# TravisWheelerLab/BATH

Measured on NVIDIA B200. Metric: frameshift Forward GCUPS, higher is better.
Workload: dtype f32

## Files before the change

### bath_b200/csrc/bathgpu.cu

```cuda
#include <cuda_runtime.h>
#include <stdint.h>
#include <stdio.h>
#include <stdarg.h>
#include <string.h>
#include <stdlib.h>
#include <math.h>
#include <thread>
#include <vector>
#include <string>
#include <algorithm>
#include <mutex>
#include <memory>

#include "../../include/bathgpu.h"
#include "fs_parser.cuh"
#include "fs_parser_v3.cuh"
#include "fs_backward.cuh"
#include "fs_domain.cuh"
#include "orf_domain.cuh"
#include "orf_filters.cuh"
#include "orf_finder.cuh"
#include "bias_filter.cuh"
#include "microbench.cuh"
#include "launch.h"
// ... 29 lines not shown
      if (ms >= 1.0) fprintf(stderr, "[bathgpu] device buffer %zu -> %zu bytes: %.2f ms\n", old, want, ms);
    }
    return BATHGPU_OK;
  }
  void release() { if (p) cudaFree(p); p = nullptr; cap = 0; }
  template <class T> T *as() const { return reinterpret_cast<T *>(p); }
};

struct FsProfileImage {
  int   which = 0, M = 0, nrows = 0, J = 0, mpad = 0, scan_steps = 5;
  DevBuf emis;
  DevBuf emis_bck, cellb3;
  DevBuf cellbmw;
  DevBuf emis_fwd;
  DevBuf cellc;
  DevBuf cellmw;
  int    mw_scan_steps = 5;
  DevBuf cellb;
  DevBuf cellf5;
  DevBuf amino;
  DevBuf oaflags;
  DevBuf oapass;
  DevBuf tfvraw;
  DevBuf zinv;
  bool  loaded = false;
};

struct FsProfileSet {
  int n = 0;
  std::vector<int> J, scan_steps, mw_scan_steps;
// ... 412 lines not shown
          for (int lane = 0; lane < 32; ++lane) {
            mw[(size_t)(5 * JW + s2) * VL + 32 * w + lane] = (lane >= d) ? (float)bsw[lane] : 0.0f;
            if (lane >= d) { biggest = std::max(biggest, bw[lane]); nbs[lane] = bsw[lane] * bsw[lane - d]; nb[lane] = bw[lane] * bw[lane - d]; }
          }
          bsw.swap(nbs); bw.swap(nb);
          if (biggest < 1.0e-9 && need == 5) need = std::max(s2, 3);
        }
        mw_scan_steps = std::max(mw_scan_steps, need);
      }
      if (getenv("BATHGPU_FULL_SCAN")) mw_scan_steps = 5;
    } else mw.clear();
    if (getenv("BATHGPU_FULL_SCAN")) scan_steps = 5;
  }
}

static void fs5_forward_consts(const Fold &f, std::vector<float> &cc)
{
  const int M = f.M, J = f.J;
  const std::vector<double> &sK = f.sK, &zK = f.zK;
  auto T = [&](int t, int k) -> double { return f.T(t, k); };
  cc.assign((size_t)(F5_COUNT * J + 5) * 32, 0.0f);
  auto C = [&](int which_c, int j, int lane) -> float & { return cc[(size_t)(which_c * J + j) * 32 + lane]; };
  std::vector<double> bfull(32, 1.0);
  for (int lane = 0; lane < 32; ++lane) {
    double pp = 1.0;
    for (int j = 0; j < J; ++j) {
      int k = lane * J + j + 1;
      if (k <= M) {
        double sn = sK[k + 1];
        C(F5_MM, j, lane) = (float)(T(tMM, k) / (zK[k] * sn));
// ... 42 lines not shown

  {
    std::vector<float> ef, cc, mw;
    forward3_tables(f, which, nrows, rfv, ef, cc, mw, im.scan_steps, im.mw_scan_steps);
    if (im.emis_fwd.reserve(ef.size() * sizeof(float)) != BATHGPU_OK) return fail(ctx, BATHGPU_EMEM, "device allocation failed");
    CUDA_TRY(ctx, cudaMemcpyAsync(im.emis_fwd.p, ef.data(), ef.size() * sizeof(float), cudaMemcpyHostToDevice, ctx->stream));
    CUDA_TRY(ctx, wait_stream(ctx));
    if (!mw.empty()) {
      if (im.cellmw.reserve(mw.size() * sizeof(float)) != BATHGPU_OK) return fail(ctx, BATHGPU_EMEM, "device allocation failed");
      CUDA_TRY(ctx, cudaMemcpyAsync(im.cellmw.p, mw.data(), mw.size() * sizeof(float), cudaMemcpyHostToDevice, ctx->stream));
      CUDA_TRY(ctx, wait_stream(ctx));
    } else im.cellmw.release();
    if (im.cellc.reserve(cc.size() * sizeof(float)) != BATHGPU_OK) return fail(ctx, BATHGPU_EMEM, "device allocation failed");
    CUDA_TRY(ctx, cudaMemcpyAsync(im.cellc.p, cc.data(), cc.size() * sizeof(float), cudaMemcpyHostToDevice, ctx->stream));
    CUDA_TRY(ctx, wait_stream(ctx));
  }

  {
    std::vector<float> cc((size_t)(BC_COUNT * J + BL_COUNT) * 32, 0.0f);
    auto C = [&](int which_c, int j, int lane) -> float & { return cc[(size_t)(which_c * J + j) * 32 + lane]; };
    std::vector<double> bfull(32, 1.0);
    for (int lane = 0; lane < 32; ++lane) {
      double pp = 1.0;
      for (int j = 0; j < J; ++j) {
        int k = lane * J + j + 1;
        if (k <= M) {
          double sn = sK[k + 1];
          C(BC_VMM, j, lane) = (float)(T(tMM, k) / (sn * zK[k]));
          C(BC_VIM, j, lane) = (float)(T(tIM, k) / sn);
          C(BC_VDM, j, lane) = (float)(T(tDM, k) / sn);
// ... 333 lines not shown
    return fail(ctx, BATHGPU_EMEM, "device allocation failed for a %lld-nt block", n);
  if (!A.bytes_valid) {
    unpack_dna4_kernel<<<(unsigned)(((n + 7) / 8 + 255) / 256), 256, 0, ctx->stream>>>(A.dna4.as<uint32_t>(), n, A.dna_bytes.as<uint8_t>());
    A.bytes_valid = true;
  }
  revcomp_kernel<<<(unsigned)((n + 255) / 256), 256, 0, ctx->stream>>>(A.dna_bytes.as<uint8_t>(), n, B.dna_bytes.as<uint8_t>());
  pack_dna4_kernel<<<(unsigned)((nwords + 255) / 256), 256, 0, ctx->stream>>>(B.dna_bytes.as<uint8_t>(), n, B.dna4.as<uint32_t>(), nwords);
  CUDA_TRY(ctx, cudaGetLastError());
  CUDA_TRY(ctx, wait_stream(ctx));
  B.block_n = n; B.nres = 0; B.bytes_valid = true;
  return BATHGPU_OK;
}


static cudaError_t dispatch_fwd(bool xmx, int J, const FsParserArgs &a, int sms, cudaStream_t s);

static int fs_fwd_block_impl(bathgpu_ctx *ctx, const uint8_t *dsq, const uint8_t *packed, int64_t n, const bathgpu_window *wins, int nwin,
                             const float xfE[2], float *fwdsc, int32_t *status)
{
  if (!ctx || (!dsq && !packed) || n < 1 || !wins || nwin < 1 || !xfE || !fwdsc || !status) return fail(ctx, BATHGPU_EINVAL, "bad arguments to bathgpu_fs_fwd_block");
  if (!ctx->fs3.loaded) return fail(ctx, BATHGPU_EINVAL, "3-codon profile not loaded");
  for (int w = 0; w < nwin; ++w)
    if (wins[w].L < 3 || wins[w].start < 1 || wins[w].start + wins[w].L - 1 > n)
      return fail(ctx, BATHGPU_EINVAL, "window %d (start %lld, L %d) is outside the block (n=%lld) or shorter than 3", w, (long long)wins[w].start, wins[w].L, (long long)n);
  CUDA_TRY(ctx, enter(ctx));
  if (!ctx->copy_stream) {
    CUDA_TRY(ctx, cudaStreamCreateWithFlags(&ctx->copy_stream, cudaStreamNonBlocking));
    CUDA_TRY(ctx, cudaStreamCreateWithFlags(&ctx->stream2, cudaStreamNonBlocking));
    for (auto &e : ctx->chunk_ev) CUDA_TRY(ctx, cudaEventCreateWithFlags(&e, cudaEventDisableTiming));
  }
// ... 54 lines not shown
  int w0 = 0, launches = 0;
  for (int c = 0; c < K; ++c) {
    const long long ready_nt = (c == K - 1) ? n : 8 * (cuts[c] / 8);
    int w1 = w0;
    while (w1 < nwin && hw[w1].start + hw[w1].L - 1 <= ready_nt) ++w1;
    if (c == K - 1) w1 = nwin;
    if (w1 == w0) continue;
    cudaStream_t s = (launches & 1) ? ctx->stream2 : ctx->stream;
    if (launches == 1) CUDA_TRY(ctx, cudaStreamWaitEvent(ctx->stream2, ctx->ev0, 0));
    CUDA_TRY(ctx, cudaStreamWaitEvent(s, pack_ev[c], 0));
    FsParserArgs a{};
    a.emis = im.emis_fwd.as<float>(); a.cellc = im.cellc.as<float>(); a.dna4 = S.dna4.as<uint32_t>();
    a.wins = ctx->wins.as<WindowDesc>() + w0; a.nwin = w1 - w0; a.mpad = im.mpad; a.tEM = xfE[0]; a.tEL = xfE[1];
    a.fwdsc = ctx->fwdsc.as<float>() + w0; a.status = ctx->status.as<int>() + w0; a.xmx = nullptr; a.xoff = nullptr;
    a.counter = ctx->counter.as<int>() + launches; a.scan_steps = im.scan_steps; a.cellmw = im.cellmw.as<float>(); a.mw_scan_steps = im.mw_scan_steps;
    CUDA_TRY(ctx, dispatch_fwd(false, im.J, a, ctx->prop.multiProcessorCount, s));
    ++launches;
    w0 = w1;
  }
  if (launches > 1) {
    CUDA_TRY(ctx, cudaEventRecord(join_ev[0], ctx->stream2));
    CUDA_TRY(ctx, cudaStreamWaitEvent(ctx->stream, join_ev[0], 0));
  }
  CUDA_TRY(ctx, cudaEventRecord(ctx->ev1, ctx->stream));
  CUDA_TRY(ctx, cudaMemcpyAsync(in_order ? fwdsc : sc.data(), ctx->fwdsc.p, (size_t)nwin * 4, cudaMemcpyDeviceToHost, ctx->stream));
  CUDA_TRY(ctx, cudaMemcpyAsync(in_order ? status : st.data(), ctx->status.p, (size_t)nwin * 4, cudaMemcpyDeviceToHost, ctx->stream));
  CUDA_TRY(ctx, wait_stream(ctx));
  CUDA_TRY(ctx, cudaStreamSynchronize(ctx->copy_stream));
  if (!in_order) for (int w = 0; w < nwin; ++w) { fwdsc[order[w]] = sc[w]; status[order[w]] = st[w]; }
  CUDA_TRY(ctx, cudaEventElapsedTime(&ctx->last_ms, ctx->ev0, ctx->ev1));
// ... 8 lines not shown
  if (!dsq) return fail(ctx, BATHGPU_EINVAL, "bad arguments to bathgpu_fs_fwd_block");
  return fs_fwd_block_impl(ctx, dsq, nullptr, n, wins, nwin, xfE, fwdsc, status);
}

extern "C" int bathgpu_fs_fwd_block_packed4(bathgpu_ctx *ctx, const uint8_t *packed, int64_t n, const bathgpu_window *wins, int nwin,
                                            const float xfE[2], float *fwdsc, int32_t *status)
{
  if (!packed) return fail(ctx, BATHGPU_EINVAL, "bad arguments to bathgpu_fs_fwd_block_packed4");
  return fs_fwd_block_impl(ctx, nullptr, packed, n, wins, nwin, xfE, fwdsc, status);
}

static int fwd_version(int J)
{
  static const int forced = [] { const char *e = getenv("BATHGPU_FWD"); int x = e ? atoi(e) : 0; return (x == 3 || x == 4) ? x : 0; }();
  if (forced) return forced;
  return (J == 10) ? 4 : 3;
}

static cudaError_t dispatch_fwd(bool xmx, int J, const FsParserArgs &a, int sms, cudaStream_t s)
{
  cudaError_t e = cudaErrorInvalidValue;
  const int v = fwd_version(J);
#define X(S) if (launch_fs3_forward_##S(J, xmx, v, a, sms, s, &e)) return e;
  BATHGPU_FOR_EACH_SET(X)
#undef X
  return cudaErrorInvalidValue;
}

static int check_windows(bathgpu_ctx *ctx, const bathgpu_window *wins, int n)
{
  for (int w = 0; w < n; ++w) {
// ... 22 lines not shown
}

extern "C" int bathgpu_fs_fwd_staged(bathgpu_ctx *ctx, const float xfE[2])
{
  if (!ctx || !xfE)          return fail(ctx, BATHGPU_EINVAL, "bad arguments to bathgpu_fs_fwd_staged");
  if (!ctx->fs3.loaded)      return fail(ctx, BATHGPU_EINVAL, "3-codon profile not loaded");
  if (ctx->nstaged < 1)      return fail(ctx, BATHGPU_EINVAL, "no windows staged");
  CUDA_TRY(ctx, enter(ctx));
  const FsProfileImage &im = ctx->fs3;
  FsParserArgs a{};
  a.emis = im.emis_fwd.as<float>(); a.cellc = im.cellc.as<float>(); a.dna4 = ctx->S().dna4.as<uint32_t>();
  a.wins = ctx->wins.as<WindowDesc>(); a.nwin = ctx->nstaged; a.mpad = im.mpad;
  a.tEM = xfE[0]; a.tEL = xfE[1];
  a.fwdsc = ctx->fwdsc.as<float>(); a.status = ctx->status.as<int>();
  a.xmx = nullptr; a.xoff = nullptr; a.counter = ctx->counter.as<int>(); a.scan_steps = im.scan_steps; a.cellmw = im.cellmw.as<float>(); a.mw_scan_steps = im.mw_scan_steps;

  CUDA_TRY(ctx, cudaMemsetAsync(ctx->counter.p, 0, 4, ctx->stream));
  CUDA_TRY(ctx, cudaEventRecord(ctx->ev0, ctx->stream));
  CUDA_TRY(ctx, dispatch_fwd(false, im.J, a, ctx->prop.multiProcessorCount, ctx->stream));
  CUDA_TRY(ctx, cudaEventRecord(ctx->ev1, ctx->stream));
  CUDA_TRY(ctx, wait_stream(ctx));
  CUDA_TRY(ctx, cudaEventElapsedTime(&ctx->last_ms, ctx->ev0, ctx->ev1));
  ctx->last_launches = 1;
  return BATHGPU_OK;
}

extern "C" int bathgpu_fetch_scores(bathgpu_ctx *ctx, float *fwdsc, int32_t *status, int n)
{
  if (!ctx || n < 1 || n > ctx->nstaged) return fail(ctx, BATHGPU_EINVAL, "bad arguments to bathgpu_fetch_scores");
  CUDA_TRY(ctx, enter(ctx));
// ... 41 lines not shown
      ctx->dmocc.reserve(rows * 4) != BATHGPU_OK || ctx->dbtot.reserve(rows * 4) != BATHGPU_OK || ctx->detot.reserve(rows * 4) != BATHGPU_OK)
    return fail(ctx, BATHGPU_EMEM, "device allocation failed for %d windows (%zu rows)", n, rows);
  CUDA_TRY(ctx, cudaMemcpyAsync(ctx->wins.p, wins, (size_t)n * sizeof(WindowDesc), cudaMemcpyHostToDevice, ctx->stream));
  CUDA_TRY(ctx, cudaMemcpyAsync(ctx->xoff.p, xoff.data(), (size_t)(n + 1) * 8, cudaMemcpyHostToDevice, ctx->stream));
  ctx->nstaged = n;
  ctx->xrows = (int64_t)rows;

  const int sms = ctx->prop.multiProcessorCount;
  CUDA_TRY(ctx, cudaEventRecord(ctx->ev0, ctx->stream));

  FsParserArgs fa{};
  fa.emis = im.emis_fwd.as<float>(); fa.cellc = im.cellc.as<float>(); fa.dna4 = ctx->S().dna4.as<uint32_t>();
  fa.wins = ctx->wins.as<WindowDesc>(); fa.nwin = n; fa.mpad = im.mpad; fa.tEM = xfE[0]; fa.tEL = xfE[1];
  fa.fwdsc = ctx->fwdsc.as<float>(); fa.status = ctx->status.as<int>();
  fa.xmx = ctx->fxmx.as<float>(); fa.xoff = ctx->xoff.as<long long>(); fa.counter = ctx->counter.as<int>(); fa.scan_steps = im.scan_steps; fa.cellmw = im.cellmw.as<float>(); fa.mw_scan_steps = im.mw_scan_steps;
  CUDA_TRY(ctx, cudaMemsetAsync(ctx->counter.p, 0, 4, ctx->stream));
  CUDA_TRY(ctx, dispatch_fwd(true, im.J, fa, sms, ctx->stream));

  FsBackwardArgs ba{};
  ba.emis = im.emis_bck.as<float>(); ba.cellb = im.cellb3.as<float>(); ba.cellbmw = im.cellbmw.as<float>(); ba.dna4 = fa.dna4; ba.wins = fa.wins; ba.nwin = n; ba.mpad = im.mpad;
  ba.tEM = xfE[0]; ba.tEL = xfE[1]; ba.fxmx = ctx->fxmx.as<float>(); ba.bxmx = ctx->bxmx.as<float>(); ba.xoff = fa.xoff;
  ba.bcksc = ctx->bcksc.as<float>(); ba.status = fa.status; ba.counter = fa.counter;
  CUDA_TRY(ctx, cudaMemsetAsync(ctx->counter.p, 0, 4, ctx->stream));
  CUDA_TRY(ctx, dispatch_bck(im.J, ba, sms, ctx->stream));

  std::vector<float> hm, hb, he;
  if (decode) {
    DomainDecodeArgs da{};
    da.fxmx = ba.fxmx; da.bxmx = ba.bxmx; da.xoff = fa.xoff; da.wins = fa.wins; da.nwin = n;
    da.tNL = xf5_loop[0]; da.tJL = xf5_loop[1]; da.tCL = xf5_loop[2];
// ... 1208 lines not shown
```

### bath_b200/csrc/fs_parser.cuh

```cuda
#pragma once
#include <cuda_runtime.h>
#include <stdint.h>

namespace bathgpu {

constexpr int kWarp = 32;

enum FwdCellConst { FC_MM = 0, FC_DM, FC_MD, FC_DD, FC_MI, FC_II, FC_COUNT };
enum FwdLaneConst { FL_B0 = 0, FL_B1, FL_B2, FL_B3, FL_B4, FL_COUNT };

struct WindowDesc {
  long long start;
  int       L;
  float     pmove;
  float     ploop;
};

struct FsSetProfile {
  const float *emis;
  const float *cellc;
  const float *cellmw;
  float        tEM, tEL;
};

// ... 3 lines not shown
  const uint32_t *dna4;
  const WindowDesc *wins;
  int             nwin;
  int             mpad;
  float           tEM, tEL;
  float          *fwdsc;
  int            *status;
  float          *xmx;
  const long long *xoff;
  int            *counter;
  int             scan_steps;
  const float    *cellmw;
  int             mw_scan_steps;
  const FsSetProfile *set;
  const int      *wprof;
};

template <int J> struct VecOf { static constexpr int V = (J % 4 == 0) ? 4 : ((J % 2 == 0) ? 2 : 1); };

__device__ __forceinline__ int codon2_fs3(int w, int x)               { int c = x * 84 + w * 21;                 return min(c, 337); }
__device__ __forceinline__ int codon3_fs3(int v, int w, int x)        { int c = x * 84 + w * 21 + v * 5 + 1;     return min(c, 336); }
__device__ __forceinline__ int codon4_fs3(int u, int v, int w, int x) { int c = x * 84 + w * 21 + v * 5 + u + 2; return min(c, 337); }

template <int J, int VEC>
__device__ __forceinline__ void load_emission_row(const float *__restrict__ row, float (&e)[J])
{
#pragma unroll
  for (int g = 0; g < J / VEC; ++g) {
    if constexpr (VEC == 4) {
      float4 t = __ldg(reinterpret_cast<const float4 *>(row) + g * kWarp);
// ... 185 lines not shown
```

### bath_b200/csrc/fs_parser_v3.cuh

```cuda
#pragma once
#include "fs_parser.cuh"

#ifndef BATHGPU_V3_JOINT_E
#define BATHGPU_V3_JOINT_E(J) (((J) >= 2 && (J) <= 5) || (J) == 8)
#endif

namespace bathgpu {

struct RowOut { float xE, xN, xJ, xC, xB, scale; };

template <int J, int VEC, int PH, int NS, bool HEAD>
__device__ __forceinline__ void fwd_row_compute(int i, int lane, FwdState<J> &S, const FwdConsts<J> &K,
                                                const char *__restrict__ emis_lane, unsigned rowbytes, uint32_t cw,
                                                float ploop, float pmove, float tEL, float tEM, RowOut &R)
{
  constexpr int P0 = PH, P1 = (PH + 3) & 3, P2 = (PH + 2) & 3, P3 = (PH + 1) & 3;
  float e2[J], e3[J], e4[J], m[J];
  load_emission_row<J, VEC>(reinterpret_cast<const float *>(emis_lane + (size_t)(cw & 511u) * rowbytes), e2);
  load_emission_row<J, VEC>(reinterpret_cast<const float *>(emis_lane + (size_t)((cw >> 9) & 511u) * rowbytes), e3);
  load_emission_row<J, VEC>(reinterpret_cast<const float *>(emis_lane + (size_t)(cw >> 18) * rowbytes), e4);

  float es0 = 0.f, es1 = 0.f;
#pragma unroll
  for (int j = 0; j < J; ++j) {
    float t = S.W[P2][j] * e4[j];
    t = fmaf(S.W[P1][j], e3[j], t);
    t = fmaf(S.W[P0][j], e2[j], t);
    m[j] = t;
    if (j == 0) es0 = t * K.qm[0]; else if (j == 1) es1 = t * K.qm[1]; else if (j & 1) es1 = fmaf(t, K.qm[j], es1); else es0 = fmaf(t, K.qm[j], es0);
  }
  float xE = warp_allsum(J > 1 ? es0 + es1 : es0);

  float A = 0.f;
#pragma unroll
  for (int j = 0; j < J; ++j) A = (j == 0) ? m[0] : fmaf(A, K.dd[j], m[j]);
// ... 17 lines not shown
    o[j] = fmaf(d, K.dm[j], t);
    if (j + 1 < J) d = fmaf(d, K.dd[j], m[j]);
    S.I[P1][j] = fmaf(S.I[P0][j], K.ii[j], m[j]);
  }
  float oprev = __shfl_up_sync(0xffffffffu, o[J - 1], 1);
  if (lane == 0) oprev = 0.f;
  S.W[P2][0] = xB + oprev;
#pragma unroll
  for (int j = 1; j < J; ++j) S.W[P2][j] = xB + o[j - 1];
  S.xN[P0] = xN; S.xJ[P0] = xJ; S.xC[P0] = xC;
  R.xE = xE; R.xN = xN; R.xJ = xJ; R.xC = xC; R.xB = xB; R.scale = 1.0f;
}

template <int J> struct RowMid { float m[J]; float es, d; };

template <int J, int VEC, int PH, int NS>
__device__ __forceinline__ void fwd_row_front(const FwdState<J> &S, const FwdConsts<J> &K, const char *__restrict__ emis_lane, unsigned rowbytes,
                                              uint32_t cw, RowMid<J> &X)
{
  constexpr int P0 = PH, P1 = (PH + 3) & 3, P2 = (PH + 2) & 3;
  float e2[J], e3[J], e4[J];
  load_emission_row<J, VEC>(reinterpret_cast<const float *>(emis_lane + (size_t)(cw & 511u) * rowbytes), e2);
  load_emission_row<J, VEC>(reinterpret_cast<const float *>(emis_lane + (size_t)((cw >> 9) & 511u) * rowbytes), e3);
  load_emission_row<J, VEC>(reinterpret_cast<const float *>(emis_lane + (size_t)(cw >> 18) * rowbytes), e4);
  float es0 = 0.f, es1 = 0.f;
#pragma unroll
  for (int j = 0; j < J; ++j) {
    float t = S.W[P2][j] * e4[j];
    t = fmaf(S.W[P1][j], e3[j], t);
    t = fmaf(S.W[P0][j], e2[j], t);
    X.m[j] = t;
    if (j == 0) es0 = t * K.qm[0]; else if (j == 1) es1 = t * K.qm[1]; else if (j & 1) es1 = fmaf(t, K.qm[j], es1); else es0 = fmaf(t, K.qm[j], es0);
  }
  X.es = (J > 1) ? es0 + es1 : es0;
  float A = 0.f;
#pragma unroll
  for (int j = 0; j < J; ++j) A = (j == 0) ? X.m[0] : fmaf(A, K.dd[j], X.m[j]);
#pragma unroll
  for (int s = 0; s < NS; ++s) {
// ... 43 lines not shown
}

template <bool XMX>
__device__ __forceinline__ void store_xrow(int i, int lane, const RowOut &R, float *__restrict__ xrow)
{
  if constexpr (XMX) {
    if (lane == 0 && i >= 0) {
      float2 *x2 = reinterpret_cast<float2 *>(xrow + (size_t)i * 6);
      x2[0] = make_float2(R.xE, R.xN);
      x2[1] = make_float2(R.xJ, R.xB);
      x2[2] = make_float2(R.xC, R.scale);
    }
  }
}

template <int J, int VEC, int PH, bool XMX, int NS, bool HEAD>
__device__ __forceinline__ void fwd_row_pair(int i, int lane, FwdState<J> &S, const FwdConsts<J> &K,
                                             const char *__restrict__ emis_lane, unsigned rowbytes, uint32_t cwA, uint32_t cwB,
                                             float ploop, float pmove, float tEL, float tEM,
                                             float &totscale, float *__restrict__ xrow)
{
  RowOut A, B;
  if constexpr (BATHGPU_V3_JOINT_E(J)) {
    RowMid<J> XA, XB;
    fwd_row_front<J, VEC, PH, NS>(S, K, emis_lane, rowbytes, cwA, XA);
    fwd_row_front<J, VEC, PH + 1, NS>(S, K, emis_lane, rowbytes, cwB, XB);
    float xEA, xEB;
    pair_allsum(lane, XA.es, XB.es, xEA, xEB);
    fwd_row_back<J, PH, HEAD>(i, lane, S, K, XA, xEA, ploop, pmove, tEL, tEM, A);
    fwd_row_back<J, PH + 1, HEAD>(i + 1, lane, S, K, XB, xEB, ploop, pmove, tEL, tEM, B);
  } else {
    fwd_row_compute<J, VEC, PH, NS, HEAD>(i, lane, S, K, emis_lane, rowbytes, cwA, ploop, pmove, tEL, tEM, A);
    fwd_row_compute<J, VEC, PH + 1, NS, HEAD>(i + 1, lane, S, K, emis_lane, rowbytes, cwB, ploop, pmove, tEL, tEM, B);
  }
  if (__builtin_expect(A.xE > 1.0e4f || B.xE > 1.0e4f, 0)) {
    if (A.xE > 1.0e4f) {
      const float sf = 1.0f / A.xE;
      scale_state<J>(S, sf);
      A.scale = A.xE; A.xN *= sf; A.xJ *= sf; A.xC *= sf; A.xB *= sf;
      B.xE *= sf; B.xN *= sf; B.xJ *= sf; B.xC *= sf; B.xB *= sf;
      totscale += logf(A.xE);
      A.xE = 1.0f;
    }
    if (B.xE > 1.0e4f) {
      const float sf = 1.0f / B.xE;
      scale_state<J>(S, sf);
      B.scale = B.xE; B.xN *= sf; B.xJ *= sf; B.xC *= sf; B.xB *= sf;
      totscale += logf(B.xE);
      B.xE = 1.0f;
    }
  }
  store_xrow<XMX>(i, lane, A, xrow);
  store_xrow<XMX>(i + 1, lane, B, xrow);
}

#ifndef BATHGPU_V3_WARPS
#define BATHGPU_V3_WARPS(J) ((J) <= 2 ? 20 : (J) == 3 ? 18 : (J) == 4 ? 16 : (J) == 5 ? 14 : (J) == 6 ? 13 : (J) == 7 ? 10 : (J) == 8 ? 9 : 8)
#endif

#ifndef BATHGPU_V3_RESIDENT
#define BATHGPU_V3_RESIDENT(J) 64
#endif

template <int J, bool XMX, int NS = 5, bool SET = false>
__global__ void __launch_bounds__(32, BATHGPU_V3_WARPS(J)) fs3_forward_parser_kernel_v3(FsParserArgs a)
{
  constexpr int VEC = VecOf<J>::V;
  const int lane = threadIdx.x & 31;

  FwdConsts<J> K;
  const char    *emis_lane = nullptr;
  float          tEM = a.tEM, tEL = a.tEL;
  int            cur = -1;
  if constexpr (!SET) {
    load_fwd_consts<J>(a.cellc, lane, K);
    emis_lane = reinterpret_cast<const char *>(a.emis + lane * VEC);
  }
  const unsigned rowbytes  = (unsigned)a.mpad * 4u;

  for (;;) {
    int w = 0;
    if (lane == 0) w = atomicAdd(a.counter, 1);
    w = __shfl_sync(0xffffffffu, w, 0);
    if (w >= a.nwin) break;
    if constexpr (SET) {
      const int p = a.wprof[w];
      if (p != cur) {
        cur = p;
        const FsSetProfile sp = a.set[p];
        load_fwd_consts<J>(sp.cellc, lane, K);
        emis_lane = reinterpret_cast<const char *>(sp.emis + lane * VEC);
        tEM = sp.tEM; tEL = sp.tEL;
// ... 11 lines not shown
    for (int r = 0; r < 4; ++r) {
#pragma unroll
      for (int j = 0; j < J; ++j) { S.W[r][j] = 0.f; S.I[r][j] = 0.f; }
      S.xN[r] = 0.f; S.xJ[r] = 0.f; S.xC[r] = 0.f;
    }
    float totscale = 0.f;

    const int nq  = (L + 4) >> 2;
    const int pad = 4 * nq - (L + 1);
    long long nib = (wd.start - 1) + (long long)(lane - pad - 3) - 1 + 8;
    uint32_t lo = __ldg(a.dna4 + (nib >> 3)), hi = __ldg(a.dna4 + (nib >> 3) + 1);
    int i = -pad;

#define BATHGPU_V3_CHUNK(HEAD_)                                                                                                   \
    {                                                                                                                             \
      const uint32_t cwl = codon_word(lo, hi, (int)(nib & 7) * 4, i + lane, L);                                                   \
      nib += 32;                                                                                                                  \
      if (q0 + 8 < nq) { lo = __ldg(a.dna4 + (nib >> 3)); hi = __ldg(a.dna4 + (nib >> 3) + 1); }                                  \
      const int qn = min(8, nq - q0);                                                                                             \
      for (int qq = 0; qq < qn; ++qq) {                                                                                           \
        const uint32_t c0 = __shfl_sync(0xffffffffu, cwl, qq * 4 + 0);                                                            \
        const uint32_t c1 = __shfl_sync(0xffffffffu, cwl, qq * 4 + 1);                                                            \
        const uint32_t c2 = __shfl_sync(0xffffffffu, cwl, qq * 4 + 2);                                                            \
        const uint32_t c3 = __shfl_sync(0xffffffffu, cwl, qq * 4 + 3);                                                            \
        fwd_row_pair<J, VEC, 0, XMX, NS, HEAD_>(i, lane, S, K, emis_lane, rowbytes, c0, c1, ploop, pmove, tEL, tEM, totscale, xrow); i += 2; \
        fwd_row_pair<J, VEC, 2, XMX, NS, HEAD_>(i, lane, S, K, emis_lane, rowbytes, c2, c3, ploop, pmove, tEL, tEM, totscale, xrow); i += 2; \
      }                                                                                                                           \
    }
    int q0 = 0;
    BATHGPU_V3_CHUNK(true)
    for (q0 = 8; q0 < nq; q0 += 8) BATHGPU_V3_CHUNK(false)
#undef BATHGPU_V3_CHUNK

    {
      float tot = S.xC[3] + S.xC[2] * ploop + S.xC[1] * ploop;
      int   st  = 0;
      float sc;
      if (isnan(tot) || isinf(tot))  { st = 16; sc = tot; }
      else if (L > 2 && tot == 0.0f) { st = 16; sc = -INFINITY; }
      else sc = totscale + logf(tot * pmove);
      if (lane == 0) { a.fwdsc[w] = sc; a.status[w] = st; }
    }
  }
}

}
```

### bath_b200/csrc/kernels_tu.cu

```cuda
#include <algorithm>
#include <cstdlib>
#include "launch.h"
#include "fs_parser.cuh"
#include "fs_parser_v3.cuh"
#include "fs_parser_v4.cuh"
#include "fs_parser_mw.cuh"
#include "fs_backward.cuh"
#include "fs_backward_mw.cuh"
#include "fs_domain.cuh"
#include "orf_domain.cuh"
#include "orf_filters.cuh"

#define FAM_FWD 1
#define FAM_BCK 2
#define FAM_FS5 3
#define FAM_ORF 4
#define FAM_FILT_MSV 5
#define FAM_FILT_VIT_LO 6
#define FAM_FILT_VIT_HI 7

#if   BATHGPU_SET == 0
#define SETNAME a
#define JLIST(X) X(1) X(2) X(3) X(4) X(5)
#elif BATHGPU_SET == 1
// ... 31 lines not shown
{
  static const int env_cap = [] { const char *e = getenv("BATHGPU_FWD_WARPS"); return e ? atoi(e) : 0; }();
  int nb = 0;
  cudaOccupancyMaxActiveBlocksPerMultiprocessor(&nb, kernel, 32, 0);
  const int cap = env_cap > 0 ? env_cap : BATHGPU_V3_RESIDENT(J);
  return std::max(1, std::min(n, sms * std::max(1, std::min(nb, cap))));
}

template <int NW, int JW, bool XMX, bool SET = false> static cudaError_t run_fwd_mw(const FsParserArgs &a, int sms, cudaStream_t s)
{
  if (a.mw_scan_steps <= 3) fs3_forward_parser_kernel_mw<NW, JW, XMX, 3, SET><<<grid_for(fs3_forward_parser_kernel_mw<NW, JW, XMX, 3, SET>, 32 * NW, 0, a.nwin, sms), 32 * NW, 0, s>>>(a);
  else                      fs3_forward_parser_kernel_mw<NW, JW, XMX, 5, SET><<<grid_for(fs3_forward_parser_kernel_mw<NW, JW, XMX, 5, SET>, 32 * NW, 0, a.nwin, sms), 32 * NW, 0, s>>>(a);
  return cudaGetLastError();
}

template <int J, bool XMX, bool SET = false> static cudaError_t run_fwd(int version, const FsParserArgs &a, int sms, cudaStream_t s)
{
  if constexpr (J >= 16) {
    static const int mw_mode = [] { const char *e = getenv("BATHGPU_FWD_MW"); return e ? atoi(e) : 1; }();
    if (version >= 3 && a.cellmw && (mw_mode >= 2 || (mw_mode == 1 && J >= 24))) return run_fwd_mw<J / kMwNodesPerLane, kMwNodesPerLane, XMX, SET>(a, sms, s);
  }
  if (version >= 4) {
    if (a.scan_steps <= 2)      fs3_forward_parser_kernel_v4<J, XMX, 2, SET><<<fwd_grid(fs3_forward_parser_kernel_v4<J, XMX, 2, SET>, J, a.nwin, sms), 32, 0, s>>>(a);
    else if (a.scan_steps == 3) fs3_forward_parser_kernel_v4<J, XMX, 3, SET><<<fwd_grid(fs3_forward_parser_kernel_v4<J, XMX, 3, SET>, J, a.nwin, sms), 32, 0, s>>>(a);
    else                        fs3_forward_parser_kernel_v4<J, XMX, 5, SET><<<fwd_grid(fs3_forward_parser_kernel_v4<J, XMX, 5, SET>, J, a.nwin, sms), 32, 0, s>>>(a);
  }
  else {
    if (a.scan_steps <= 2)      fs3_forward_parser_kernel_v3<J, XMX, 2, SET><<<fwd_grid(fs3_forward_parser_kernel_v3<J, XMX, 2, SET>, J, a.nwin, sms), 32, 0, s>>>(a);
    else if (a.scan_steps == 3) fs3_forward_parser_kernel_v3<J, XMX, 3, SET><<<fwd_grid(fs3_forward_parser_kernel_v3<J, XMX, 3, SET>, J, a.nwin, sms), 32, 0, s>>>(a);
    else                        fs3_forward_parser_kernel_v3<J, XMX, 5, SET><<<fwd_grid(fs3_forward_parser_kernel_v3<J, XMX, 5, SET>, J, a.nwin, sms), 32, 0, s>>>(a);
  }
  return cudaGetLastError();
}
bool CAT(launch_fs3_forward_set_, SETNAME)(int J, int version, const FsParserArgs &a, int sms, cudaStream_t s, cudaError_t *err)
{
  switch (J) {
#define X(J_) case J_: *err = run_fwd<J_, false, true>(version, a, sms, s); return true;
  JLIST(X)
#undef X
  default: return false;
  }
}
bool CAT(launch_fs3_forward_, SETNAME)(int J, bool xmx, int version, const FsParserArgs &a, int sms, cudaStream_t s, cudaError_t *err)
{
  switch (J) {
#define X(J_) case J_: *err = xmx ? run_fwd<J_, true>(version, a, sms, s) : run_fwd<J_, false>(version, a, sms, s); return true;
  JLIST(X)
#undef X
  default: return false;
  }
}
void CAT(preload_fwd_, SETNAME)(int J)
{
  switch (J) {
#define X(J_) case J_: touch(fs3_forward_parser_kernel_v3<J_, false, 2>); touch(fs3_forward_parser_kernel_v3<J_, true, 2>); touch(fs3_forward_parser_kernel_v3<J_, false, 3>); \
                       touch(fs3_forward_parser_kernel_v3<J_, true, 3>); touch(fs3_forward_parser_kernel_v3<J_, false, 5>); touch(fs3_forward_parser_kernel_v3<J_, true, 5>); \
                       if (J_ == 10) { touch(fs3_forward_parser_kernel_v4<J_, false, 2>); touch(fs3_forward_parser_kernel_v4<J_, true, 2>); touch(fs3_forward_parser_kernel_v4<J_, false, 3>); \
                                       touch(fs3_forward_parser_kernel_v4<J_, true, 3>); touch(fs3_forward_parser_kernel_v4<J_, false, 5>); touch(fs3_forward_parser_kernel_v4<J_, true, 5>); } \
                       break;
  JLIST(X)
#undef X
  default: break;
  }
}
#endif

#if BATHGPU_FAMILY == FAM_BCK
template <int J> static cudaError_t run_bck(const FsBackwardArgs &a, int sms, cudaStream_t s)
{
  if constexpr (J >= 16) {
    static const int mw_mode = [] { const char *e = getenv("BATHGPU_BCK_MW"); return e ? atoi(e) : 1; }();
// ... 248 lines not shown
```

### bath_b200/csrc/launch.h

```cpp
#pragma once
#include <cuda_runtime.h>

namespace bathgpu {

struct FsParserArgs;
struct FsBackwardArgs;
struct DomainArgs;
struct TraceArgs;
struct OrfDomainArgs;
struct OrfFwdArgs;
struct FilterArgs;

#define BATHGPU_FOR_EACH_SET(X) X(a) X(b) X(c) X(d) X(e) X(f)

#define BATHGPU_DECLARE_SET(S)                                                                                                       \
  bool launch_fs3_forward_##S(int J, bool xmx, int version, const FsParserArgs &a, int sms, cudaStream_t s, cudaError_t *err);       \
  bool launch_fs3_backward_##S(int J, const FsBackwardArgs &a, int sms, cudaStream_t s, cudaError_t *err);                           \
  bool launch_fs5_domains_##S(int J, const DomainArgs &a, const TraceArgs &t, int sms, cudaStream_t s, cudaError_t *err);            \
  bool launch_fs5_forward_matrix_##S(int J, const DomainArgs &a, int sms, cudaStream_t s, cudaError_t *err);                         \
  bool launch_orf_domains_##S(int J, bool full, const OrfDomainArgs &a, const TraceArgs &t, int sms, cudaStream_t s, cudaError_t *err); \
  bool launch_orf_forward_matrix_##S(int J, const OrfDomainArgs &a, int sms, cudaStream_t s, cudaError_t *err);                            \
  bool launch_orf_forward_parser_##S(int J, const OrfFwdArgs &a, int sms, cudaStream_t s, cudaError_t *err);                        \
  bool launch_fs3_forward_set_##S(int J, int version, const FsParserArgs &a, int sms, cudaStream_t s, cudaError_t *err);            \
  bool launch_fs5_forward_set_##S(int J, const DomainArgs &a, int sms, cudaStream_t s, cudaError_t *err);                            \
  void preload_fwd_##S(int J); void preload_bck_##S(int J); void preload_fs5_##S(int J); void preload_orf_##S(int J);
BATHGPU_FOR_EACH_SET(BATHGPU_DECLARE_SET)
#undef BATHGPU_DECLARE_SET

constexpr int kMwNodesPerLane = 8;

bool launch_msv_filter(int W, int P, int mode, const FilterArgs &a, int sms, cudaStream_t s, cudaError_t *err);
bool launch_vit_filter_lo(int P, const FilterArgs &a, int sms, cudaStream_t s, cudaError_t *err);
bool launch_vit_filter_hi(int P, const FilterArgs &a, int sms, cudaStream_t s, cudaError_t *err);
void preload_msv_filter(int W, int P); void preload_vit_filter_lo(int P); void preload_vit_filter_hi(int P);

}
```

Measured before the change: 1339.

## Serve forward emission rows for 2- and 3-nt codons from Blackwell TMEM

For the 3-codon forward parser with J between 2 and 8, the host deduplicates identical emission rows for the 2- and 3-nucleotide codon classes. It packs them into a per-lane column image that each CTA copies into tensor memory at startup, and a remap table rewrites codon words to the deduplicated slots. The inner loop then reads the e2/e3 rows with tcgen05.ld instead of global/L1 loads, and 4-nt emissions come from a compacted table. This adds TMEM allocation and fill per block, multi-warp CTAs, and padded shared memory to cap how many blocks co-reside, which may reduce occupancy.

```diff
diff --git a/bath_b200/csrc/bathgpu.cu b/bath_b200/csrc/bathgpu.cu
--- a/bath_b200/csrc/bathgpu.cu
+++ b/bath_b200/csrc/bathgpu.cu
@@ -67,6 +67,10 @@
   DevBuf cellbmw;
   DevBuf emis_fwd;
   DevBuf cellc;
+  DevBuf tm_src;
+  DevBuf emis4;
+  DevBuf cmap;
+  int    tm_n = 0, tm_cols = 0;
   DevBuf cellmw;
   int    mw_scan_steps = 5;
   DevBuf cellb;
@@ -509,6 +513,44 @@
   }
 }
 
+static int forward3_tmem_image(const std::vector<float> &ef, int J, int mpad, std::vector<float> &tm, std::vector<float> &e4,
+                               std::vector<uint32_t> &cmap, int &tm_n)
+{
+  std::vector<int> rep23, rep4;
+  auto slot = [&](std::vector<int> &rep, int c) -> uint32_t {
+    for (size_t r = 0; r < rep.size(); ++r)
+      if (memcmp(&ef[(size_t)rep[r] * mpad], &ef[(size_t)c * mpad], (size_t)mpad * sizeof(float)) == 0) return (uint32_t)r;
+    rep.push_back(c);
+    return (uint32_t)(rep.size() - 1);
+  };
+  cmap.assign(338, 0u);
+  for (int c = 0; c < 338; ++c) {
+    const int r = c % 21;
+    const bool nt23 = c >= 336 || r == 0 || r % 5 == 1, nt4 = c == 337 || (c < 336 && r != 0 && r % 5 != 1);
+    if (nt23) cmap[c] |= slot(rep23, c);
+    if (nt4)  cmap[c] |= slot(rep4, c) << 16;
+  }
+  tm_n = (int)rep23.size();
+  const int cols = tm_n * J <= 256 ? 256 : tm_n * J <= 512 ? 512 : 0;
+  if (!cols) return 0;
+  tm.assign((size_t)tm_n * J * 32, 0.0f);
+  for (int s = 0; s < tm_n; ++s) {
+    int P = 0;
+    for (int c = 8; c >= 1; c >>= 1) {
+      if (!(J & c)) continue;
+      for (int i = 0; i < c; ++i) {
+        const int col = tm_n * P + s * c + i;
+        if (col >= tm_n * J || col >= cols) return 0;
+        for (int lane = 0; lane < 32; ++lane) tm[(size_t)col * 32 + lane] = ef[(size_t)rep23[s] * mpad + perm_index(lane * J + P + i, J)];
+      }
+      P += c;
+    }
+  }
+  e4.resize(rep4.size() * (size_t)mpad);
+  for (size_t r = 0; r < rep4.size(); ++r) memcpy(&e4[r * mpad], &ef[(size_t)rep4[r] * mpad], (size_t)mpad * sizeof(float));
+  return cols;
+}
+
 static void fs5_forward_consts(const Fold &f, std::vector<float> &cc)
 {
   const int M = f.M, J = f.J;
@@ -581,6 +623,22 @@
     if (im.cellc.reserve(cc.size() * sizeof(float)) != BATHGPU_OK) return fail(ctx, BATHGPU_EMEM, "device allocation failed");
     CUDA_TRY(ctx, cudaMemcpyAsync(im.cellc.p, cc.data(), cc.size() * sizeof(float), cudaMemcpyHostToDevice, ctx->stream));
     CUDA_TRY(ctx, wait_stream(ctx));
+    im.tm_cols = 0; im.tm_n = 0;
+    if (which == 3 && J >= 2 && J <= 8) {
+      std::vector<float> tm, e4;
+      std::vector<uint32_t> cmap;
+      const int cols = forward3_tmem_image(ef, J, mpad, tm, e4, cmap, im.tm_n);
+      if (cols) {
+        if (im.tm_src.reserve(tm.size() * sizeof(float)) != BATHGPU_OK || im.emis4.reserve(e4.size() * sizeof(float)) != BATHGPU_OK ||
+            im.cmap.reserve(cmap.size() * sizeof(uint32_t)) != BATHGPU_OK)
+          return fail(ctx, BATHGPU_EMEM, "device allocation failed");
+        CUDA_TRY(ctx, cudaMemcpyAsync(im.tm_src.p, tm.data(), tm.size() * sizeof(float), cudaMemcpyHostToDevice, ctx->stream));
+        CUDA_TRY(ctx, cudaMemcpyAsync(im.emis4.p, e4.data(), e4.size() * sizeof(float), cudaMemcpyHostToDevice, ctx->stream));
+        CUDA_TRY(ctx, cudaMemcpyAsync(im.cmap.p, cmap.data(), cmap.size() * sizeof(uint32_t), cudaMemcpyHostToDevice, ctx->stream));
+        CUDA_TRY(ctx, wait_stream(ctx));
+        im.tm_cols = cols;
+      }
+    }
   }
 
   {
@@ -944,6 +1002,11 @@
 
 
 static cudaError_t dispatch_fwd(bool xmx, int J, const FsParserArgs &a, int sms, cudaStream_t s);
+static void set_tmem_args(const FsProfileImage &im, FsParserArgs &a)
+{
+  if (!im.tm_cols) return;
+  a.tm_src = im.tm_src.as<float>(); a.emis4 = im.emis4.as<float>(); a.cmap = im.cmap.as<uint32_t>(); a.tm_n = im.tm_n; a.tm_cols = im.tm_cols;
+}
 
 static int fs_fwd_block_impl(bathgpu_ctx *ctx, const uint8_t *dsq, const uint8_t *packed, int64_t n, const bathgpu_window *wins, int nwin,
                              const float xfE[2], float *fwdsc, int32_t *status)
@@ -1028,6 +1091,7 @@
     a.wins = ctx->wins.as<WindowDesc>() + w0; a.nwin = w1 - w0; a.mpad = im.mpad; a.tEM = xfE[0]; a.tEL = xfE[1];
     a.fwdsc = ctx->fwdsc.as<float>() + w0; a.status = ctx->status.as<int>() + w0; a.xmx = nullptr; a.xoff = nullptr;
     a.counter = ctx->counter.as<int>() + launches; a.scan_steps = im.scan_steps; a.cellmw = im.cellmw.as<float>(); a.mw_scan_steps = im.mw_scan_steps;
+    set_tmem_args(im, a);
     CUDA_TRY(ctx, dispatch_fwd(false, im.J, a, ctx->prop.multiProcessorCount, s));
     ++launches;
     w0 = w1;
@@ -1066,7 +1130,7 @@
 {
   static const int forced = [] { const char *e = getenv("BATHGPU_FWD"); int x = e ? atoi(e) : 0; return (x == 3 || x == 4) ? x : 0; }();
   if (forced) return forced;
-  return (J == 10) ? 4 : 3;
+  return (J == 10) ? 4 : (J >= 2 && J <= 8) ? kFwdTmem : 3;
 }
 
 static cudaError_t dispatch_fwd(bool xmx, int J, const FsParserArgs &a, int sms, cudaStream_t s)
@@ -1119,6 +1183,7 @@
   a.tEM = xfE[0]; a.tEL = xfE[1];
   a.fwdsc = ctx->fwdsc.as<float>(); a.status = ctx->status.as<int>();
   a.xmx = nullptr; a.xoff = nullptr; a.counter = ctx->counter.as<int>(); a.scan_steps = im.scan_steps; a.cellmw = im.cellmw.as<float>(); a.mw_scan_steps = im.mw_scan_steps;
+  set_tmem_args(im, a);
 
   CUDA_TRY(ctx, cudaMemsetAsync(ctx->counter.p, 0, 4, ctx->stream));
   CUDA_TRY(ctx, cudaEventRecord(ctx->ev0, ctx->stream));
@@ -1190,6 +1255,7 @@
   fa.wins = ctx->wins.as<WindowDesc>(); fa.nwin = n; fa.mpad = im.mpad; fa.tEM = xfE[0]; fa.tEL = xfE[1];
   fa.fwdsc = ctx->fwdsc.as<float>(); fa.status = ctx->status.as<int>();
   fa.xmx = ctx->fxmx.as<float>(); fa.xoff = ctx->xoff.as<long long>(); fa.counter = ctx->counter.as<int>(); fa.scan_steps = im.scan_steps; fa.cellmw = im.cellmw.as<float>(); fa.mw_scan_steps = im.mw_scan_steps;
+  set_tmem_args(im, fa);
   CUDA_TRY(ctx, cudaMemsetAsync(ctx->counter.p, 0, 4, ctx->stream));
   CUDA_TRY(ctx, dispatch_fwd(true, im.J, fa, sms, ctx->stream));
 
diff --git a/bath_b200/csrc/fs_parser.cuh b/bath_b200/csrc/fs_parser.cuh
--- a/bath_b200/csrc/fs_parser.cuh
+++ b/bath_b200/csrc/fs_parser.cuh
@@ -41,6 +41,11 @@
   int             mw_scan_steps;
   const FsSetProfile *set;
   const int      *wprof;
+  const float    *tm_src;
+  const float    *emis4;
+  const uint32_t *cmap;
+  int             tm_n;
+  int             tm_cols;
 };
 
 template <int J> struct VecOf { static constexpr int V = (J % 4 == 0) ? 4 : ((J % 2 == 0) ? 2 : 1); };
diff --git a/bath_b200/csrc/fs_parser_v3.cuh b/bath_b200/csrc/fs_parser_v3.cuh
--- a/bath_b200/csrc/fs_parser_v3.cuh
+++ b/bath_b200/csrc/fs_parser_v3.cuh
@@ -1,5 +1,6 @@
 #pragma once
 #include "fs_parser.cuh"
+#include "fs_tmem.cuh"
 
 #ifndef BATHGPU_V3_JOINT_E
 #define BATHGPU_V3_JOINT_E(J) (((J) >= 2 && (J) <= 5) || (J) == 8)
@@ -9,16 +10,13 @@
 
 struct RowOut { float xE, xN, xJ, xC, xB, scale; };
 
-template <int J, int VEC, int PH, int NS, bool HEAD>
+template <int J, int PH, int NS, bool HEAD>
 __device__ __forceinline__ void fwd_row_compute(int i, int lane, FwdState<J> &S, const FwdConsts<J> &K,
-                                                const char *__restrict__ emis_lane, unsigned rowbytes, uint32_t cw,
+                                                const float (&e2)[J], const float (&e3)[J], const float (&e4)[J],
                                                 float ploop, float pmove, float tEL, float tEM, RowOut &R)
 {
   constexpr int P0 = PH, P1 = (PH + 3) & 3, P2 = (PH + 2) & 3, P3 = (PH + 1) & 3;
-  float e2[J], e3[J], e4[J], m[J];
-  load_emission_row<J, VEC>(reinterpret_cast<const float *>(emis_lane + (size_t)(cw & 511u) * rowbytes), e2);
-  load_emission_row<J, VEC>(reinterpret_cast<const float *>(emis_lane + (size_t)((cw >> 9) & 511u) * rowbytes), e3);
-  load_emission_row<J, VEC>(reinterpret_cast<const float *>(emis_lane + (size_t)(cw >> 18) * rowbytes), e4);
+  float m[J];
 
   float es0 = 0.f, es1 = 0.f;
 #pragma unroll
@@ -66,15 +64,11 @@
 
 template <int J> struct RowMid { float m[J]; float es, d; };
 
-template <int J, int VEC, int PH, int NS>
-__device__ __forceinline__ void fwd_row_front(const FwdState<J> &S, const FwdConsts<J> &K, const char *__restrict__ emis_lane, unsigned rowbytes,
-                                              uint32_t cw, RowMid<J> &X)
+template <int J, int PH, int NS>
+__device__ __forceinline__ void fwd_row_front(const FwdState<J> &S, const FwdConsts<J> &K,
+                                              const float (&e2)[J], const float (&e3)[J], const float (&e4)[J], RowMid<J> &X)
 {
   constexpr int P0 = PH, P1 = (PH + 3) & 3, P2 = (PH + 2) & 3;
-  float e2[J], e3[J], e4[J];
-  load_emission_row<J, VEC>(reinterpret_cast<const float *>(emis_lane + (size_t)(cw & 511u) * rowbytes), e2);
-  load_emission_row<J, VEC>(reinterpret_cast<const float *>(emis_lane + (size_t)((cw >> 9) & 511u) * rowbytes), e3);
-  load_emission_row<J, VEC>(reinterpret_cast<const float *>(emis_lane + (size_t)(cw >> 18) * rowbytes), e4);
   float es0 = 0.f, es1 = 0.f;
 #pragma unroll
   for (int j = 0; j < J; ++j) {
@@ -148,24 +142,38 @@
   }
 }
 
-template <int J, int VEC, int PH, bool XMX, int NS, bool HEAD>
+template <int J, int VEC, int PH, bool XMX, int NS, bool HEAD, bool TM>
 __device__ __forceinline__ void fwd_row_pair(int i, int lane, FwdState<J> &S, const FwdConsts<J> &K,
-                                             const char *__restrict__ emis_lane, unsigned rowbytes, uint32_t cwA, uint32_t cwB,
-                                             float ploop, float pmove, float tEL, float tEM,
+                                             const char *__restrict__ emis_lane, unsigned rowbytes, uint32_t tmq, uint32_t tmn,
+                                             uint32_t cwA, uint32_t cwB, float ploop, float pmove, float tEL, float tEM,
                                              float &totscale, float *__restrict__ xrow)
 {
+  float e2A[J], e3A[J], e4A[J], e2B[J], e3B[J], e4B[J];
+  if constexpr (TM) {
+    tm_ld_pair<J>(tmq, tmn, cwA, cwB, e2A, e3A, e2B, e3B);
+  } else {
+    load_emission_row<J, VEC>(reinterpret_cast<const float *>(emis_lane + (size_t)(cwA & 511u) * rowbytes), e2A);
+    load_emission_row<J, VEC>(reinterpret_cast<const float *>(emis_lane + (size_t)((cwA >> 9) & 511u) * rowbytes), e3A);
+  }
+  load_emission_row<J, VEC>(reinterpret_cast<const float *>(emis_lane + (size_t)(cwA >> 18) * rowbytes), e4A);
+  if constexpr (!TM) {
+    load_emission_row<J, VEC>(reinterpret_cast<const float *>(emis_lane + (size_t)(cwB & 511u) * rowbytes), e2B);
+    load_emission_row<J, VEC>(reinterpret_cast<const float *>(emis_lane + (size_t)((cwB >> 9) & 511u) * rowbytes), e3B);
+  }
+  load_emission_row<J, VEC>(reinterpret_cast<const float *>(emis_lane + (size_t)(cwB >> 18) * rowbytes), e4B);
+
   RowOut A, B;
   if constexpr (BATHGPU_V3_JOINT_E(J)) {
     RowMid<J> XA, XB;
-    fwd_row_front<J, VEC, PH, NS>(S, K, emis_lane, rowbytes, cwA, XA);
-    fwd_row_front<J, VEC, PH + 1, NS>(S, K, emis_lane, rowbytes, cwB, XB);
+    fwd_row_front<J, PH, NS>(S, K, e2A, e3A, e4A, XA);
+    fwd_row_front<J, PH + 1, NS>(S, K, e2B, e3B, e4B, XB);
     float xEA, xEB;
     pair_allsum(lane, XA.es, XB.es, xEA, xEB);
     fwd_row_back<J, PH, HEAD>(i, lane, S, K, XA, xEA, ploop, pmove, tEL, tEM, A);
     fwd_row_back<J, PH + 1, HEAD>(i + 1, lane, S, K, XB, xEB, ploop, pmove, tEL, tEM, B);
   } else {
-    fwd_row_compute<J, VEC, PH, NS, HEAD>(i, lane, S, K, emis_lane, rowbytes, cwA, ploop, pmove, tEL, tEM, A);
-    fwd_row_compute<J, VEC, PH + 1, NS, HEAD>(i + 1, lane, S, K, emis_lane, rowbytes, cwB, ploop, pmove, tEL, tEM, B);
+    fwd_row_compute<J, PH, NS, HEAD>(i, lane, S, K, e2A, e3A, e4A, ploop, pmove, tEL, tEM, A);
+    fwd_row_compute<J, PH + 1, NS, HEAD>(i + 1, lane, S, K, e2B, e3B, e4B, ploop, pmove, tEL, tEM, B);
   }
   if (__builtin_expect(A.xE > 1.0e4f || B.xE > 1.0e4f, 0)) {
     if (A.xE > 1.0e4f) {
@@ -196,9 +204,15 @@
 #define BATHGPU_V3_RESIDENT(J) 64
 #endif
 
-template <int J, bool XMX, int NS = 5, bool SET = false>
-__global__ void __launch_bounds__(32, BATHGPU_V3_WARPS(J)) fs3_forward_parser_kernel_v3(FsParserArgs a)
-{
+#define BATHGPU_V3_TM_BLOCKS(J) ((J) == 6 ? 2 : 1)
+#define BATHGPU_V3_TM_WARPS(J)  ((J) == 6 ? 8 : BATHGPU_V3_WARPS(J))
+
+template <int J, bool XMX, int NS = 5, bool SET = false, bool TM = false>
+__global__ void __launch_bounds__(TM ? 32 * BATHGPU_V3_TM_WARPS(J) : 32, TM ? BATHGPU_V3_TM_BLOCKS(J) : BATHGPU_V3_WARPS(J))
+fs3_forward_parser_kernel_v3(FsParserArgs a)
+{
+  static_assert(!(TM && SET), "the set path reads the full tables");
+  static_assert(!TM || BATHGPU_V3_TM_WARPS(J) >= 4, "warps 0-3 fill the four TMEM lane quarters");
   constexpr int VEC = VecOf<J>::V;
   const int lane = threadIdx.x & 31;
 
@@ -206,10 +220,13 @@
   const char    *emis_lane = nullptr;
   float          tEM = a.tEM, tEL = a.tEL;
   int            cur = -1;
+  uint32_t       tmbase = 0, tmq = 0;
+  const uint32_t tmn = (uint32_t)a.tm_n;
   if constexpr (!SET) {
     load_fwd_consts<J>(a.cellc, lane, K);
-    emis_lane = reinterpret_cast<const char *>(a.emis + lane * VEC);
-  }
+    emis_lane = reinterpret_cast<const char *>((TM ? a.emis4 : a.emis) + lane * VEC);
+  }
+  if constexpr (TM) tmq = tm_alloc_fill(a.tm_src, a.tm_n * J, a.tm_cols, tmbase);
   const unsigned rowbytes  = (unsigned)a.mpad * 4u;
 
   for (;;) {
@@ -251,7 +268,8 @@
 
 #define BATHGPU_V3_CHUNK(HEAD_)                                                                                                   \
     {                                                                                                                             \
-      const uint32_t cwl = codon_word(lo, hi, (int)(nib & 7) * 4, i + lane, L);                                                   \
+      uint32_t cwl = codon_word(lo, hi, (int)(nib & 7) * 4, i + lane, L);                                                         \
+      if constexpr (TM) cwl = tm_codon_word(cwl, a.cmap);                                                                         \
       nib += 32;                                                                                                                  \
       if (q0 + 8 < nq) { lo = __ldg(a.dna4 + (nib >> 3)); hi = __ldg(a.dna4 + (nib >> 3) + 1); }                                  \
       const int qn = min(8, nq - q0);                                                                                             \
@@ -260,8 +278,10 @@
         const uint32_t c1 = __shfl_sync(0xffffffffu, cwl, qq * 4 + 1);                                                            \
         const uint32_t c2 = __shfl_sync(0xffffffffu, cwl, qq * 4 + 2);                                                            \
         const uint32_t c3 = __shfl_sync(0xffffffffu, cwl, qq * 4 + 3);                                                            \
-        fwd_row_pair<J, VEC, 0, XMX, NS, HEAD_>(i, lane, S, K, emis_lane, rowbytes, c0, c1, ploop, pmove, tEL, tEM, totscale, xrow); i += 2; \
-        fwd_row_pair<J, VEC, 2, XMX, NS, HEAD_>(i, lane, S, K, emis_lane, rowbytes, c2, c3, ploop, pmove, tEL, tEM, totscale, xrow); i += 2; \
+        fwd_row_pair<J, VEC, 0, XMX, NS, HEAD_, TM>(i, lane, S, K, emis_lane, rowbytes, tmq, tmn, c0, c1, ploop, pmove, tEL, tEM, totscale, xrow); \
+        i += 2;                                                                                                                   \
+        fwd_row_pair<J, VEC, 2, XMX, NS, HEAD_, TM>(i, lane, S, K, emis_lane, rowbytes, tmq, tmn, c2, c3, ploop, pmove, tEL, tEM, totscale, xrow); \
+        i += 2;                                                                                                                   \
       }                                                                                                                           \
     }
     int q0 = 0;
@@ -279,6 +299,7 @@
       if (lane == 0) { a.fwdsc[w] = sc; a.status[w] = st; }
     }
   }
-}
-
-}
+  if constexpr (TM) tm_free(tmbase, a.tm_cols);
+}
+
+}
diff --git a/bath_b200/csrc/fs_tmem.cuh b/bath_b200/csrc/fs_tmem.cuh
--- /dev/null
+++ b/bath_b200/csrc/fs_tmem.cuh
@@ -0,0 +1,91 @@
+#pragma once
+#include "fs_parser.cuh"
+
+namespace bathgpu {
+
+__device__ __forceinline__ uint32_t tm_codon_word(uint32_t cw, const uint32_t *__restrict__ cmap)
+{
+  return (__ldg(cmap + (cw & 511u)) & 0xffffu) | ((__ldg(cmap + ((cw >> 9) & 511u)) & 0xffffu) << 9) | ((__ldg(cmap + (cw >> 18)) >> 16) << 18);
+}
+
+__device__ __forceinline__ uint32_t tm_alloc_fill(const float *__restrict__ src, int ncols_used, int ncols, uint32_t &base)
+{
+  __shared__ uint32_t tm_base;
+  const int warp = threadIdx.x >> 5, lane = threadIdx.x & 31;
+  if (warp == 0) {
+    asm volatile("tcgen05.alloc.cta_group::1.sync.aligned.shared::cta.b32 [%0], %1;"
+                 :: "r"((uint32_t)__cvta_generic_to_shared(&tm_base)), "r"(ncols) : "memory");
+    asm volatile("tcgen05.relinquish_alloc_permit.cta_group::1.sync.aligned;" ::: "memory");
+  }
+  asm volatile("tcgen05.fence::before_thread_sync;" ::: "memory");
+  __syncthreads();
+  asm volatile("tcgen05.fence::after_thread_sync;" ::: "memory");
+  base = tm_base;
+  const uint32_t quarter = base + ((uint32_t)(32 * (warp & 3)) << 16);
+  if (warp < 4) {
+    for (int c = 0; c < ncols_used; ++c) {
+      const uint32_t v = __float_as_uint(__ldg(src + (size_t)c * kWarp + lane));
+      asm volatile("tcgen05.st.sync.aligned.32x32b.x1.b32 [%0], {%1};" :: "r"(quarter + (uint32_t)c), "r"(v) : "memory");
+    }
+    asm volatile("tcgen05.wait::st.sync.aligned;" ::: "memory");
+  }
+  asm volatile("tcgen05.fence::before_thread_sync;" ::: "memory");
+  __syncthreads();
+  asm volatile("tcgen05.fence::after_thread_sync;" ::: "memory");
+  return quarter;
+}
+
+__device__ __forceinline__ void tm_free(uint32_t base, int ncols)
+{
+  asm volatile("tcgen05.fence::before_thread_sync;" ::: "memory");
+  __syncthreads();
+  asm volatile("tcgen05.fence::after_thread_sync;" ::: "memory");
+  if ((threadIdx.x >> 5) == 0) asm volatile("tcgen05.dealloc.cta_group::1.sync.aligned.b32 %0, %1;" :: "r"(base), "r"(ncols) : "memory");
+}
+
+template <int J, int C, int P>
+__device__ __forceinline__ void tm_ld_digit(uint32_t quarter, uint32_t slot, uint32_t n, uint32_t (&r)[J])
+{
+  if constexpr ((J & C) != 0) {
+    const uint32_t ta = quarter + n * (uint32_t)P + slot * (uint32_t)C;
+    if constexpr (C == 8)
+      asm volatile("tcgen05.ld.sync.aligned.32x32b.x8.b32 {%0, %1, %2, %3, %4, %5, %6, %7}, [%8];"
+                   : "=r"(r[P]), "=r"(r[P + 1]), "=r"(r[P + 2]), "=r"(r[P + 3]), "=r"(r[P + 4]), "=r"(r[P + 5]), "=r"(r[P + 6]), "=r"(r[P + 7]) : "r"(ta));
+    else if constexpr (C == 4)
+      asm volatile("tcgen05.ld.sync.aligned.32x32b.x4.b32 {%0, %1, %2, %3}, [%4];" : "=r"(r[P]), "=r"(r[P + 1]), "=r"(r[P + 2]), "=r"(r[P + 3]) : "r"(ta));
+    else if constexpr (C == 2)
+      asm volatile("tcgen05.ld.sync.aligned.32x32b.x2.b32 {%0, %1}, [%2];" : "=r"(r[P]), "=r"(r[P + 1]) : "r"(ta));
+    else
+      asm volatile("tcgen05.ld.sync.aligned.32x32b.x1.b32 {%0}, [%1];" : "=r"(r[P]) : "r"(ta));
+  }
+}
+
+template <int J>
+__device__ __forceinline__ void tm_ld_row(uint32_t quarter, uint32_t slot, uint32_t n, uint32_t (&r)[J])
+{
+  static_assert(J >= 1 && J < 16, "TMEM rows: J < 16");
+  tm_ld_digit<J, 8, 0>(quarter, slot, n, r);
+  tm_ld_digit<J, 4, (J & 8)>(quarter, slot, n, r);
+  tm_ld_digit<J, 2, (J & 12)>(quarter, slot, n, r);
+  tm_ld_digit<J, 1, (J & 14)>(quarter, slot, n, r);
+}
+
+template <int J>
+__device__ __forceinline__ void tm_ld_pair(uint32_t quarter, uint32_t n, uint32_t cwA, uint32_t cwB,
+                                           float (&e2A)[J], float (&e3A)[J], float (&e2B)[J], float (&e3B)[J])
+{
+  uint32_t r2A[J], r3A[J], r2B[J], r3B[J];
+  tm_ld_row<J>(quarter, cwA & 511u, n, r2A);
+  tm_ld_row<J>(quarter, (cwA >> 9) & 511u, n, r3A);
+  tm_ld_row<J>(quarter, cwB & 511u, n, r2B);
+  tm_ld_row<J>(quarter, (cwB >> 9) & 511u, n, r3B);
+  asm volatile("tcgen05.wait::ld.sync.aligned;" ::: "memory");
+#pragma unroll
+  for (int j = 0; j < J; ++j) {
+    asm volatile("" : "+r"(r2A[j]), "+r"(r3A[j]), "+r"(r2B[j]), "+r"(r3B[j]));
+    e2A[j] = __uint_as_float(r2A[j]); e3A[j] = __uint_as_float(r3A[j]);
+    e2B[j] = __uint_as_float(r2B[j]); e3B[j] = __uint_as_float(r3B[j]);
+  }
+}
+
+}
diff --git a/bath_b200/csrc/kernels_tu.cu b/bath_b200/csrc/kernels_tu.cu
--- a/bath_b200/csrc/kernels_tu.cu
+++ b/bath_b200/csrc/kernels_tu.cu
@@ -69,13 +69,43 @@
   return cudaGetLastError();
 }
 
+template <int J, bool XMX, int NS> static cudaError_t launch_fwd_tm(const FsParserArgs &a, int sms, cudaStream_t s)
+{
+  auto kernel = fs3_forward_parser_kernel_v3<J, XMX, NS, false, true>;
+  constexpr int warps = BATHGPU_V3_TM_WARPS(J);
+  const int cap = 512 / a.tm_cols;
+  int nb = 0, dev = 0, smem_sm = 0, smem_res = 0;
+  cudaError_t e;
+  if ((e = cudaOccupancyMaxActiveBlocksPerMultiprocessor(&nb, kernel, 32 * warps, 0)) != cudaSuccess) return e;
+  size_t smem = 0;
+  if (nb > cap) {
+    if ((e = cudaGetDevice(&dev)) != cudaSuccess) return e;
+    if ((e = cudaDeviceGetAttribute(&smem_sm, cudaDevAttrMaxSharedMemoryPerMultiprocessor, dev)) != cudaSuccess) return e;
+    if ((e = cudaDeviceGetAttribute(&smem_res, cudaDevAttrReservedSharedMemoryPerBlock, dev)) != cudaSuccess) return e;
+    smem = (size_t)(smem_sm / (cap + 1) - smem_res + 1024);
+    if ((e = cudaFuncSetAttribute(kernel, cudaFuncAttributeMaxDynamicSharedMemorySize, (int)smem)) != cudaSuccess) return e;
+    if ((e = cudaOccupancyMaxActiveBlocksPerMultiprocessor(&nb, kernel, 32 * warps, smem)) != cudaSuccess) return e;
+  }
+  if (nb < 1 || nb > cap) return cudaErrorInvalidConfiguration;
+  const int blocks = std::max(1, std::min((a.nwin + warps - 1) / warps, sms * nb));
+  kernel<<<blocks, 32 * warps, smem, s>>>(a);
+  return cudaGetLastError();
+}
+
 template <int J, bool XMX, bool SET = false> static cudaError_t run_fwd(int version, const FsParserArgs &a, int sms, cudaStream_t s)
 {
+  if constexpr (!SET && J >= 2 && J <= 8) {
+    if (version == kFwdTmem && a.tm_src) {
+      if (a.scan_steps <= 2)      return launch_fwd_tm<J, XMX, 2>(a, sms, s);
+      else if (a.scan_steps == 3) return launch_fwd_tm<J, XMX, 3>(a, sms, s);
+      else                        return launch_fwd_tm<J, XMX, 5>(a, sms, s);
+    }
+  }
   if constexpr (J >= 16) {
     static const int mw_mode = [] { const char *e = getenv("BATHGPU_FWD_MW"); return e ? atoi(e) : 1; }();
     if (version >= 3 && a.cellmw && (mw_mode >= 2 || (mw_mode == 1 && J >= 24))) return run_fwd_mw<J / kMwNodesPerLane, kMwNodesPerLane, XMX, SET>(a, sms, s);
   }
-  if (version >= 4) {
+  if (version == 4) {
     if (a.scan_steps <= 2)      fs3_forward_parser_kernel_v4<J, XMX, 2, SET><<<fwd_grid(fs3_forward_parser_kernel_v4<J, XMX, 2, SET>, J, a.nwin, sms), 32, 0, s>>>(a);
     else if (a.scan_steps == 3) fs3_forward_parser_kernel_v4<J, XMX, 3, SET><<<fwd_grid(fs3_forward_parser_kernel_v4<J, XMX, 3, SET>, J, a.nwin, sms), 32, 0, s>>>(a);
     else                        fs3_forward_parser_kernel_v4<J, XMX, 5, SET><<<fwd_grid(fs3_forward_parser_kernel_v4<J, XMX, 5, SET>, J, a.nwin, sms), 32, 0, s>>>(a);
@@ -105,11 +135,20 @@
   default: return false;
   }
 }
+template <int J> static void touch_fwd_tm()
+{
+  if constexpr (J >= 2 && J <= 8) {
+    touch(fs3_forward_parser_kernel_v3<J, false, 2, false, true>); touch(fs3_forward_parser_kernel_v3<J, true, 2, false, true>);
+    touch(fs3_forward_parser_kernel_v3<J, false, 3, false, true>); touch(fs3_forward_parser_kernel_v3<J, true, 3, false, true>);
+    touch(fs3_forward_parser_kernel_v3<J, false, 5, false, true>); touch(fs3_forward_parser_kernel_v3<J, true, 5, false, true>);
+  }
+}
 void CAT(preload_fwd_, SETNAME)(int J)
 {
   switch (J) {
 #define X(J_) case J_: touch(fs3_forward_parser_kernel_v3<J_, false, 2>); touch(fs3_forward_parser_kernel_v3<J_, true, 2>); touch(fs3_forward_parser_kernel_v3<J_, false, 3>); \
                        touch(fs3_forward_parser_kernel_v3<J_, true, 3>); touch(fs3_forward_parser_kernel_v3<J_, false, 5>); touch(fs3_forward_parser_kernel_v3<J_, true, 5>); \
+                       touch_fwd_tm<J_>();                                                                                                                   \
                        if (J_ == 10) { touch(fs3_forward_parser_kernel_v4<J_, false, 2>); touch(fs3_forward_parser_kernel_v4<J_, true, 2>); touch(fs3_forward_parser_kernel_v4<J_, false, 3>); \
                                        touch(fs3_forward_parser_kernel_v4<J_, true, 3>); touch(fs3_forward_parser_kernel_v4<J_, false, 5>); touch(fs3_forward_parser_kernel_v4<J_, true, 5>); } \
                        break;
diff --git a/bath_b200/csrc/launch.h b/bath_b200/csrc/launch.h
--- a/bath_b200/csrc/launch.h
+++ b/bath_b200/csrc/launch.h
@@ -27,6 +27,8 @@
 BATHGPU_FOR_EACH_SET(BATHGPU_DECLARE_SET)
 #undef BATHGPU_DECLARE_SET
 
+constexpr int kFwdTmem = 5;
+
 constexpr int kMwNodesPerLane = 8;
 
 bool launch_msv_filter(int W, int P, int mode, const FilterArgs &a, int sms, cudaStream_t s, cudaError_t *err);
```

Measured after the change: 1126 (median of 6 runs). 0.841x the previous value.
